# tobwei/APTAI

Hardware: AMD Instinct MI355X
Metric: utterances/sec (10 s @ 16 kHz) train-step (higher is better)
Workload: dtype bf16

## Files before the change

### aptai_amd/csrc/gemm.hip

```cpp
#include <stdlib.h>

#include <mutex>
#include <set>
#include <type_traits>

#include "common.h"
#include "gemm_common.h"

using namespace aptai_gemm;

namespace {

#ifdef APTAI_STAMPS
__device__ unsigned long long g_stamps[4096 * 8];
#define APTAI_STAMP(slot)                                                                          \
    do {                                                                                           \
        if (threadIdx.x == 0 && blockIdx.x < 4096 && blockIdx.y == 0 && blockIdx.z == 0)           \
            g_stamps[blockIdx.x * 8 + (slot)] = wall_clock64();                                    \
    } while (0)
extern "C" int aptai_debug_read_stamps(void* host_out) {
    return hipMemcpyFromSymbol(host_out, HIP_SYMBOL(g_stamps), sizeof(g_stamps)) == hipSuccess ? 0 : 1;
}
#else
#define APTAI_STAMP(slot) do {} while (0)
#endif

void epi_trace(const GemmArgs& g, int tile) {
    static const bool on = getenv("APTAI_EPI_TRACE") != nullptr;
    if (!on) return;
    static std::mutex mu;
    static std::set<int> seen;
    const int w = g.flags | (g.out_pre ? EPX_PRE : 0) | (g.colscale_n > 0 ? EPX_CS : 0);
    std::lock_guard<std::mutex> lk(mu);
    if (!seen.insert(w).second) return;
    bool listed = false;
#define APTAI_EPI_CASE(W) listed = listed || (w == (W));
    APTAI_EPI_WORDS(APTAI_EPI_CASE)
#undef APTAI_EPI_CASE
    fprintf(stderr, "[aptai epi] flag word 0x%x (tile %d, %d x %d x %d): %s\n", w, tile, g.M, g.N, g.K, listed ? "compiled" : "RUN-TIME form");
}

template <bool A_KM, bool B_KM, bool OUT_F32, int BM_T = 128, bool ROWSUM = false>
__device__ __forceinline__ void gemm_tile_body(GemmArgs g, const int bid, const int batch, const int split, float* rowsum = nullptr) {
    extern __shared__ __attribute__((aligned(16))) char smem[];
    APTAI_STAMP(0);
    const int tid = threadIdx.x;
    const int lane = tid & 63;
    const int wave = __builtin_amdgcn_readfirstlane(tid >> 6);
    const int wm = wave >> 1, wn = wave & 1;

    int tile_m, tile_n;
    raster2d(bid, g.tiles_m, g.tiles_n, g.raster_gm, tile_m, tile_n);
    constexpr int NI = BM_T / 32;
    constexpr int WM = BM_T / 2;
    constexpr int NA_IT = BM_T / 32;
    constexpr int A_BYTES_T = BM_T * BK * 2;
    constexpr int STAGE_T = A_BYTES_T + BN * BK * 2;
    constexpr int NPASS = BM_T / 16;
    static_assert(BM_T == 128 || (BM_T == 64 && !A_KM), "64-row tiles are built for K-contiguous A only");
    constexpr bool RING5 = A_KM && B_KM;
    const int m0 = tile_m * BM_T, n0 = tile_n * BN;

    if (batch >= 0) batch_offset<OUT_F32>(g, batch / g.nb_inner, batch % g.nb_inner);
    const auto [kt_begin, nk] = splitk_range(g, split);

    f32x4 acc[NI][4];
#pragma unroll
    for (int i = 0; i < NI; ++i)
#pragma unroll
        for (int j = 0; j < 4; ++j) acc[i][j] = (f32x4){0.f, 0.f, 0.f, 0.f};

    static_assert(!ROWSUM || (RING5 && OUT_F32), "row sums ride on the ring loop of the K-major fp32 weight-gradient tile");
    const bool rs_wave = ROWSUM && rowsum != nullptr && tile_n == 0 && wn == 0;
    const bf16x8 ones8 = __builtin_bit_cast(bf16x8, (short8v){0x3f80, 0x3f80, 0x3f80, 0x3f80, 0x3f80, 0x3f80, 0x3f80, 0x3f80});
    f32x4 racc[ROWSUM ? NI : 1];
#pragma unroll
    for (int i = 0; i < (ROWSUM ? NI : 1); ++i) racc[i] = (f32x4){0.f, 0.f, 0.f, 0.f};

    const int wave_base_tid = wave * 64;
    const bool wave_active = (m0 + wm * WM < g.M) && (n0 + wn * 64 < g.N);
    const bf16_t* pa[NA_IT];
    const bf16_t* pb[4];
    const long stepA = A_KM ? (long)BK * g.lda : (long)BK, stepB = B_KM ? (long)BK * g.ldb : (long)BK;
#pragma unroll
    for (int it = 0; it < NA_IT; ++it) pa[it] = stage_src<A_KM>(g.A, g.lda, m0, g.M, it, tid) + kt_begin * stepA;
#pragma unroll
    for (int it = 0; it < 4; ++it) pb[it] = stage_src<B_KM>(g.B, g.ldb, n0, g.N, it, tid) + kt_begin * stepB;
    auto stage = [&](char* buf) {
        char* dst = buf + wave_base_tid * 16;
#pragma unroll
        for (int it = 0; it < NA_IT; ++it) {
            __builtin_amdgcn_global_load_lds(GLB_PTR(pa[it]), LDS_PTR(dst + it * (NTHREADS * 16)), 16, 0, 0);
            pa[it] += stepA;
        }
#pragma unroll
        for (int it = 0; it < 4; ++it) {
            __builtin_amdgcn_global_load_lds(GLB_PTR(pb[it]), LDS_PTR(dst + A_BYTES_T + it * (NTHREADS * 16)), 16, 0, 0);
            pb[it] += stepB;
        }
    };
    if constexpr (RING5) {
        constexpr int HALF_T = RING_HALF_BYTES;
        const bf16_t* ha[2];
        const bf16_t* hb[2];
        const long hstepA = 32 * (long)g.lda, hstepB = 32 * (long)g.ldb;
#pragma unroll
        for (int it = 0; it < 2; ++it) {
// ... 650 lines not shown
        int cfirst = c - 1;
        while (cfirst > 0 && (int)((unsigned)cfirst * (unsigned)total / (unsigned)G) > tile * KT) --cfirst;
        if (tid == 0) {
            bool ok = true;
            for (int cp = cfirst; cp < c && ok; ++cp) {
                unsigned spins = 0;
                while (__hip_atomic_load(sk.flags + cp, __ATOMIC_RELAXED, __HIP_MEMORY_SCOPE_AGENT) == 0u) {
                    if (++spins > SK_SPIN_LIMIT) { atomicExch(sk.status, 1u); ok = false; break; }
                    __builtin_amdgcn_s_sleep(2);
                }
            }
            __builtin_amdgcn_fence(__ATOMIC_ACQUIRE, "agent");
            asm volatile("s_waitcnt vmcnt(0)" ::: "memory");
        }
        __syncthreads();
        {
            constexpr int QI = 8;
            const int nq = 4 * (c - cfirst);
            auto issue_quarter = [&](int q) {
                const float* slab = sk.slabs + (long)(cfirst + (q >> 2)) * SK_SLAB_FLOATS;
                char* dst = smem + (q & 1) * (QI * T2_THREADS * 16);
#pragma unroll
                for (int e = 0; e < QI; ++e) {
                    const int idx = (q & 3) * QI + e;
                    __builtin_amdgcn_global_load_lds(GLB_PTR(slab + ((long)idx * T2_THREADS + tid) * 4),
                                                     LDS_PTR(dst + (e * T2_THREADS + wave_base_tid) * 16), 16, 0, 0);
                }
            };
            issue_quarter(0);
            if (nq > 1) issue_quarter(1);
            for (int q = 0; q < nq; ++q) {
                if (q + 1 < nq) asm volatile("s_waitcnt vmcnt(8)" ::: "memory");
                else asm volatile("s_waitcnt vmcnt(0)" ::: "memory");
                const char* src = smem + (q & 1) * (QI * T2_THREADS * 16);
                f32x4 part[QI];
#pragma unroll
                for (int e = 0; e < QI; ++e) part[e] = *(const f32x4*)(src + (e * T2_THREADS + tid) * 16);
                asm volatile("s_waitcnt lgkmcnt(0)" ::: "memory");
                if (q + 2 < nq) issue_quarter(q + 2);
#pragma unroll
                for (int a = 0; a < 2; ++a)
#pragma unroll
                    for (int b = 0; b < 2; ++b)
#pragma unroll
                        for (int i = 0; i < 4; ++i)
#pragma unroll
                            for (int j = 0; j < 2; ++j) {
                                const int idx = ((a * 2 + b) * 4 + i) * 2 + j;
                                if ((idx >> 3) == (q & 3)) acc[a][b][i][j] += part[idx & 7];
                            }
            }
            __syncthreads();
        }
        if (tid == 0)
            for (int cp = cfirst; cp < c; ++cp) __hip_atomic_store(sk.flags + cp, 0u, __ATOMIC_RELAXED, __HIP_MEMORY_SCOPE_AGENT);
        gemm256_epilogue<OUT_F32>(g, smem, m0, n0, 0, acc, tid, lane, wr, wc);
    }
}

constexpr int SK_MAX_GRID = 256;
constexpr int64_t SK_HEADER_BYTES = 4096;
static inline int64_t sk_workspace_bytes() { return SK_HEADER_BYTES + (int64_t)SK_MAX_GRID * SK_SLAB_FLOATS * 4; }

template <bool A_KM, bool B_KM, bool OUT_F32>
int launch_gemm256_sk(const GemmArgs& g, void* ws, hipStream_t stream) {
    SkArgs sk;
    sk.status = (unsigned*)ws;
    sk.flags = (unsigned*)((char*)ws + 256);
    sk.slabs = (float*)((char*)ws + SK_HEADER_BYTES);
    sk.kt_per_tile = g.K / BK;
    const long total = (long)g.tiles_m * g.tiles_n * sk.kt_per_tile;
    if (total >= (1L << 23)) APTAI_FAIL(APTAI_ERR_INVALID, "aptai_gemm_bf16: stream-K iteration count %ld out of range", total);
    sk.total_iters = (int)total;
    const int grid = total < SK_MAX_GRID ? (int)total : SK_MAX_GRID;
    return launch_kernel<gemm256_sk_kernel<A_KM, B_KM, OUT_F32>>({T2_THREADS, T2_SMEM, "gemm256_sk_kernel"}, dim3(grid), stream, g, sk);
}

constexpr int T3_THREADS = 512;
constexpr int T3_BM = 128, T3_BN = 192;
constexpr int T3_A_BYTES = T3_BM * BK * 2;
constexpr int T3_B_BYTES = T3_BN * BK * 2;
constexpr int T3_STAGE = T3_A_BYTES + T3_B_BYTES;
constexpr int T3_SMEM = 3 * T3_STAGE;
constexpr int T3_EPI_PITCH = T3_BN * 4 + 16;
static_assert(T3_BM * T3_EPI_PITCH <= T3_SMEM, "epilogue tile must fit the staging LDS");

__device__ __forceinline__ int pn_swz(int krow) { return (((krow >> 1) & 1) | (((krow >> 3) & 1) << 1)) << 1; }

template <bool KM>
__device__ __forceinline__ const bf16_t* stage3_src(const bf16_t* __restrict__ base, long ld, int row0, int rows_total, int it,
                                                    int tid) {
    if (!KM) {
        const int slot = it * T3_THREADS + tid, row = slot >> 3, pc = slot & 7;
        int grow = row0 + row;
        grow = grow < rows_total ? grow : rows_total - 1;
        return base + (long)grow * ld + ((pc ^ (row & 7)) << 3);
    } else {
        const int krow = tid >> 3, pc = tid & 7;
        int col = row0 + it * 64 + ((pc ^ pn_swz(krow)) << 3);
        col = col <= rows_total - 8 ? col : rows_total - 8;
        return base + (long)krow * ld + col;
    }
}

template <bool KM>
__device__ __forceinline__ bf16x8 read_frag3(const char* lds_tile, int row_base, int ks, int lane) {
    if (!KM) {
        return read_frag(lds_tile, row_base, ks, lane);
    } else {
        const char* panel = lds_tile + (row_base >> 6) * 8192;
        const int rb = row_base & 63;
        const int gq = lane >> 4, i = lane & 15, qq = i >> 2, p = i & 3;
        const int ch = (rb >> 3) + (p >> 1);
        const int sub = (p & 1) << 3;
        const int k_lo = ks * 32 + gq * 8 + qq;
        const int k_hi = k_lo + 4;
        const char* a0 = panel + k_lo * 128 + ((ch ^ pn_swz(k_lo)) << 4) + sub;
        const char* a1 = panel + k_hi * 128 + ((ch ^ pn_swz(k_hi)) << 4) + sub;
        short4v lo = __builtin_amdgcn_ds_read_tr16_b64_v4i16((__attribute__((address_space(3))) short4v*)a0);
        short4v hi = __builtin_amdgcn_ds_read_tr16_b64_v4i16((__attribute__((address_space(3))) short4v*)a1);
        short8v r = {lo[0], lo[1], lo[2], lo[3], hi[0], hi[1], hi[2], hi[3]};
        return __builtin_bit_cast(bf16x8, r);
    }
}

template <bool A_KM, bool B_KM, bool OUT_F32>
__global__ __launch_bounds__(T3_THREADS, 1) void gemm192_kernel(GemmArgs g) {
    extern __shared__ __attribute__((aligned(16))) char smem[];
    APTAI_STAMP(0);
    const int tid = threadIdx.x;
    const int lane = tid & 63;
    const int wave = __builtin_amdgcn_readfirstlane(tid >> 6);
    const int wm = wave >> 2, wn = wave & 3;
    const int wave_base_tid = wave * 64;

    const int nwg = g.tiles_m * g.tiles_n;
    const int bid = xcd_remap(blockIdx.x, nwg);
    int tile_m, tile_n;
    raster2d(bid, g.tiles_m, g.tiles_n, g.raster_gm, tile_m, tile_n);
    const int m0 = tile_m * T3_BM, n0 = tile_n * T3_BN;
    if (gridDim.y > 1) batch_offset<OUT_F32>(g, blockIdx.y / g.nb_inner, blockIdx.y % g.nb_inner);
    const int split = blockIdx.z;
    const auto [kt_begin, nk] = splitk_range(g, split);

    const bf16_t* pa[2];
    const bf16_t* pb[3];
    const long stepA = A_KM ? (long)BK * g.lda : (long)BK;
    const long stepB = B_KM ? (long)BK * g.ldb : (long)BK;
#pragma unroll
    for (int it = 0; it < 2; ++it) pa[it] = stage3_src<A_KM>(g.A, g.lda, m0, g.M, it, tid) + (long)kt_begin * stepA;
#pragma unroll
    for (int it = 0; it < 3; ++it) pb[it] = stage3_src<B_KM>(g.B, g.ldb, n0, g.N, it, tid) + (long)kt_begin * stepB;
    auto stage = [&](int slot) {
        char* buf = smem + slot * T3_STAGE + wave_base_tid * 16;
#pragma unroll
        for (int it = 0; it < 2; ++it) {
            __builtin_amdgcn_global_load_lds(GLB_PTR(pa[it]), LDS_PTR(buf + it * (T3_THREADS * 16)), 16, 0, 0);
            pa[it] += stepA;
        }
#pragma unroll
        for (int it = 0; it < 3; ++it) {
            __builtin_amdgcn_global_load_lds(GLB_PTR(pb[it]), LDS_PTR(buf + T3_A_BYTES + it * (T3_THREADS * 16)), 16, 0, 0);
            pb[it] += stepB;
        }
    };

    f32x4 acc[4][3];
#pragma unroll
    for (int i = 0; i < 4; ++i)
#pragma unroll
        for (int j = 0; j < 3; ++j) acc[i][j] = (f32x4){0.f, 0.f, 0.f, 0.f};

    if constexpr (!A_KM && B_KM) {
        u32x4 aa[2][4];
        short4v bl[2][3], bh[2][3];
        auto read_half = [&](int slot, int ks) {
            const char* sa = smem + slot * T3_STAGE;
            const char* sb = sa + T3_A_BYTES;
#pragma unroll
            for (int i = 0; i < 4; ++i) {
                const int row = wm * 64 + i * 16 + (lane & 15), q = ks * 4 + (lane >> 4);
                const uint32_t addr = lds_u32(sa) + (uint32_t)(row * 128 + ((q ^ (row & 7)) << 4));
                asm volatile("ds_read_b128 %0, %1" : "=v"(aa[ks][i]) : "v"(addr));
            }
#pragma unroll
            for (int j = 0; j < 3; ++j) {
                const int row_base = wn * 48 + j * 16;
                const char* panel = sb + (row_base >> 6) * 8192;
                const int rb = row_base & 63;
                const int gq = lane >> 4, li = lane & 15, qq = li >> 2, pp = li & 3;
                const int ch = (rb >> 3) + (pp >> 1);
                const int sub = (pp & 1) << 3;
                const int k_lo = ks * 32 + gq * 8 + qq, k_hi = k_lo + 4;
                const uint32_t a0 = lds_u32(panel) + (uint32_t)(k_lo * 128 + ((ch ^ pn_swz(k_lo)) << 4) + sub);
                const uint32_t a1 = lds_u32(panel) + (uint32_t)(k_hi * 128 + ((ch ^ pn_swz(k_hi)) << 4) + sub);
                asm volatile("ds_read_b64_tr_b16 %0, %1" : "=v"(bl[ks][j]) : "v"(a0));
                asm volatile("ds_read_b64_tr_b16 %0, %1" : "=v"(bh[ks][j]) : "v"(a1));
            }
        };
        auto mfma_half = [&](int ks) {
#pragma unroll
            for (int i = 0; i < 4; ++i)
#pragma unroll
                for (int j = 0; j < 3; ++j)
                    acc[i][j] = __builtin_amdgcn_mfma_f32_16x16x32_bf16(combine_tr(bl[ks][j], bh[ks][j]), __builtin_bit_cast(bf16x8, aa[ks][i]),
                                                                        acc[i][j], 0, 0, 0);
        };
#define APTAI_TIE_HALF(K) "+v"(aa[K][0]), "+v"(aa[K][1]), "+v"(aa[K][2]), "+v"(aa[K][3]), "+v"(bl[K][0]), "+v"(bl[K][1]), "+v"(bl[K][2]), \
                          "+v"(bh[K][0]), "+v"(bh[K][1]), "+v"(bh[K][2])
        if (nk > 0) {
            stage(0);
            if (nk > 1) stage(1);
            if (nk > 2) stage(2);
            if (nk > 2) asm volatile("s_waitcnt vmcnt(10)" ::: "memory");
            else if (nk > 1) asm volatile("s_waitcnt vmcnt(5)" ::: "memory");
            else asm volatile("s_waitcnt vmcnt(0)" ::: "memory");
            __builtin_amdgcn_s_barrier();
            asm volatile("" ::: "memory");
            read_half(0, 0);
            read_half(0, 1);
        }
        int cur = 0;
        for (int kt = 0; kt < nk; ++kt) {
            const int nxt = cur == 2 ? 0 : cur + 1;
            asm volatile("s_waitcnt lgkmcnt(10)" : APTAI_TIE_HALF(0));
            mfma_half(0);
            if (kt + 1 < nk) {
                if (kt + 2 < nk) asm volatile("s_waitcnt vmcnt(5) lgkmcnt(0)" ::: "memory");
                else asm volatile("s_waitcnt vmcnt(0) lgkmcnt(0)" ::: "memory");
                __builtin_amdgcn_s_barrier();
                asm volatile("" ::: "memory");
                if (kt + 3 < nk) stage(cur);
                asm volatile("" : APTAI_TIE_HALF(1));
                read_half(nxt, 0);
            } else {
                asm volatile("s_waitcnt lgkmcnt(0)" : APTAI_TIE_HALF(1));
            }
            mfma_half(1);
            if (kt + 1 < nk) read_half(nxt, 1);
            cur = nxt;
        }
#undef APTAI_TIE_HALF
    } else {
    bf16x8 af[2][4], bfr[2][3];
    auto read_half = [&](int slot, int ks) {
        const char* sa = smem + slot * T3_STAGE;
        const char* sb = sa + T3_A_BYTES;
#pragma unroll
        for (int i = 0; i < 4; ++i) af[ks][i] = read_frag3<A_KM>(sa, wm * 64 + i * 16, ks, lane);
#pragma unroll
        for (int j = 0; j < 3; ++j) bfr[ks][j] = read_frag3<B_KM>(sb, wn * 48 + j * 16, ks, lane);
    };
    auto mfma_half = [&](int ks) {
#pragma unroll
        for (int i = 0; i < 4; ++i)
#pragma unroll
            for (int j = 0; j < 3; ++j)
                acc[i][j] = __builtin_amdgcn_mfma_f32_16x16x32_bf16(bfr[ks][j], af[ks][i], acc[i][j], 0, 0, 0);
    };

    if (nk > 0) {
        stage(0);
        if (nk > 1) stage(1);
        if (nk > 2) stage(2);
        if (nk > 2) asm volatile("s_waitcnt vmcnt(10)" ::: "memory");
        else if (nk > 1) asm volatile("s_waitcnt vmcnt(5)" ::: "memory");
        else asm volatile("s_waitcnt vmcnt(0)" ::: "memory");
        __builtin_amdgcn_s_barrier();
        asm volatile("" ::: "memory");
        read_half(0, 0);
        read_half(0, 1);
    }
    int cur = 0;
#ifdef APTAI_STAMPS
    unsigned long long seg[5] = {0, 0, 0, 0, 0}, tp = __builtin_amdgcn_s_memtime();
#define SEG(i) do { const unsigned long long tn = __builtin_amdgcn_s_memtime(); seg[i] += tn - tp; tp = tn; } while (0)
#else
#define SEG(i) do {} while (0)
#endif
    for (int kt = 0; kt < nk; ++kt) {
        const int nxt = cur == 2 ? 0 : cur + 1;
        mfma_half(0);
        SEG(0);
        if (kt + 1 < nk) {
            if (kt + 2 < nk) asm volatile("s_waitcnt vmcnt(5) lgkmcnt(0)" ::: "memory");
            else asm volatile("s_waitcnt vmcnt(0) lgkmcnt(0)" ::: "memory");
            __builtin_amdgcn_s_barrier();
            asm volatile("" ::: "memory");
            SEG(1);
            if (kt + 3 < nk) stage(cur);
            read_half(nxt, 0);
            SEG(2);
        }
        mfma_half(1);
        SEG(3);
        if (kt + 1 < nk) read_half(nxt, 1);
        SEG(4);
        cur = nxt;
    }
#ifdef APTAI_STAMPS
    if (threadIdx.x == 0 && blockIdx.x < 4096 && blockIdx.y == 0 && blockIdx.z == 0) {
        g_stamps[blockIdx.x * 8 + 1] = seg[0];
        g_stamps[blockIdx.x * 8 + 5] = seg[1];
        g_stamps[blockIdx.x * 8 + 6] = seg[2];
        g_stamps[blockIdx.x * 8 + 7] = seg[3] | (seg[4] << 32);
    }
#endif
#undef SEG
    }
    asm volatile("s_waitcnt vmcnt(0) lgkmcnt(0)" ::: "memory");
    __syncthreads();

    APTAI_STAMP(2);
    int tid_e, lane_e, m0_e, n0_e;
    epi_idx(tid, lane, m0, n0, tid_e, lane_e, m0_e, n0_e);
    const int fx = epi_flag_word(g);
    auto body = [&](auto w) {
        constexpr int FM = decltype(w)::value;
        const int flags = FM >= 0 ? FM : fx;
        u32x4 resv[6], auxv[6];
    #pragma unroll
        for (int pass = 0; pass < 6; ++pass) {
            resv[pass] = (u32x4){0u, 0u, 0u, 0u};
            auxv[pass] = (u32x4){0u, 0u, 0u, 0u};
        }
        if (!OUT_F32 && (flags & (APTAI_EPI_RESIDUAL | APTAI_EPI_DGELU | APTAI_EPI_MUL_AUX))) {
    #pragma unroll
            for (int pass = 0; pass < 6; ++pass) {
                const int c = pass * T3_THREADS + tid_e, ml = c / 24, cl = (c - ml * 24) * 8;
                int m = m0_e + ml, n = n0_e + cl;
                m = m < g.M ? m : g.M - 1;
                n = n <= g.N - 8 ? n : g.N - 8;
                if (flags & APTAI_EPI_RESIDUAL) resv[pass] = *(const u32x4*)(g.residual + (long)m * g.ldr + n);
                if (flags & (APTAI_EPI_DGELU | APTAI_EPI_MUL_AUX)) auxv[pass] = *(const u32x4*)(g.aux + (long)m * g.ldaux + n);
            }
        }
    #pragma unroll
        for (int i = 0; i < 4; ++i) {
            const int ml = wm * 64 + i * 16 + (lane_e & 15);
    #pragma unroll
            for (int j = 0; j < 3; ++j) {
                const int nl = wn * 48 + j * 16 + (lane_e >> 4) * 4;
                *(f32x4*)(smem + ml * T3_EPI_PITCH + nl * 4) = acc[i][j];
            }
        }
        __syncthreads();
        const float alpha = (flags & APTAI_EPI_ALPHA) ? g.alpha : 1.0f;
        uint32_t sd0 = g.seed0, sd1 = g.seed1;
        if (flags & APTAI_EPI_DROPOUT) apply_salt(g.salt, sd0, sd1);
    #pragma unroll
        for (int pass = 0; pass < 6; ++pass) {
            const int c = pass * T3_THREADS + tid_e, ml = c / 24, cl = (c - ml * 24) * 8;
            const int m = m0_e + ml, n = n0_e + cl;
            if (m >= g.M || n >= g.N) continue;
            const f32x4 v0 = *(const f32x4*)(smem + ml * T3_EPI_PITCH + cl * 4);
            const f32x4 v1 = *(const f32x4*)(smem + ml * T3_EPI_PITCH + cl * 4 + 16);
            float v[8] = {v0[0], v0[1], v0[2], v0[3], v1[0], v1[1], v1[2], v1[3]};
            if (flags & APTAI_EPI_BIAS) {
                const f32x4 b0 = *(const f32x4*)(g.bias + n), b1 = *(const f32x4*)(g.bias + n + 4);
    #pragma unroll
                for (int r = 0; r < 4; ++r) { v[r] = fmaf(v[r], alpha, b0[r]); v[4 + r] = fmaf(v[4 + r], alpha, b1[r]); }
            } else if (flags & APTAI_EPI_ALPHA) {
    #pragma unroll
                for (int r = 0; r < 8; ++r) v[r] *= alpha;
            }
            if (OUT_F32) {
                store_f32_tail(g, flags, v, m, n, split);
                continue;
            }
            epilogue_chunk<FM>(v, g, flags, (long)m, n, auxv[pass], resv[pass], sd0, sd1);
            __builtin_amdgcn_sched_barrier(0);
        }
    };
    if (OUT_F32) body(EpiWord<-1>{});
    else epi_dispatch(fx, body);
    APTAI_STAMP(3);
#ifdef APTAI_STAMPS
    asm volatile("s_waitcnt vmcnt(0)" ::: "memory");
    APTAI_STAMP(4);
#endif
}

}


struct GemmKnobs {
    int tile;
    double f256;
    int m64;
    int raster;
    bool splitn;
    bool epi_runtime;
};
static const GemmKnobs& gemm_knobs() {
    static const auto env = [](const char* name, const char* unset) { const char* e = getenv(name); return e ? e : unset; };
    static const GemmKnobs k = {atoi(env("APTAI_GEMM_TILE", "0")), atof(env("APTAI_GEMM_F256", "1.25")), atoi(env("APTAI_GEMM_M64", "1")),
                                atoi(env("APTAI_GEMM_RASTER", "-1")), atoi(env("APTAI_GEMM_SPLITN", "0")) != 0 && !getenv("APTAI_GEMM_TILE"),
                                atoi(env("APTAI_EPI_RUNTIME", "0")) != 0};
    return k;
}
static int raster_group(const GemmKnobs& k, int entry_default) { return k.raster >= 0 ? k.raster : entry_default; }

struct GemmPlan : aptai_gemm_plan_info { const char* refusal; };
static constexpr int tile_rows(int t) { return t == 64 ? 64 : (t == 256 || t == 257) ? T2_BM : t == 448 ? 256 : t == 192 ? T3_BM : BM; }
static constexpr int tile_cols(int t) { return t == 192 ? T3_BN : (t == 256 || t == 257) ? T2_BN : t == 448 ? 192 : BN; }
static void launch_shape(const aptai_gemm_desc& d, int& nbatch, int& nsplit, int& ktiles_per_split) {
    nbatch = (d.batch_outer > 1 || d.batch_inner > 1) ? (d.batch_outer > 0 ? d.batch_outer : 1) * (d.batch_inner > 0 ? d.batch_inner : 1) : 1;
    const int total_kt = (int)(d.K / BK);
    nsplit = d.split_k > 0 ? (d.split_k < total_kt ? d.split_k : total_kt) : 1;
    ktiles_per_split = (int)ceil_div(total_kt, nsplit);
    nsplit = (int)ceil_div(total_kt, ktiles_per_split);
}

static int validate_desc(const aptai_gemm_desc* d) {
    APTAI_REQUIRE(d != nullptr, "aptai_gemm_bf16: null descriptor");
    APTAI_REQUIRE(d->M > 0 && d->N > 0 && d->K > 0, "aptai_gemm_bf16: empty problem M=%ld N=%ld K=%ld", (long)d->M,
                  (long)d->N, (long)d->K);
    APTAI_REQUIRE(d->K % BK == 0, "aptai_gemm_bf16: K=%ld must be a multiple of %d", (long)d->K, BK);
    APTAI_REQUIRE(d->N % 8 == 0, "aptai_gemm_bf16: N=%ld must be a multiple of 8", (long)d->N);
    APTAI_REQUIRE(d->A && d->B && d->C, "aptai_gemm_bf16: null operand");
    APTAI_REQUIRE(d->lda % 8 == 0 && d->ldb % 8 == 0 && d->ldc % 8 == 0, "aptai_gemm_bf16: leading dims must keep 16-B alignment");
    if (d->residual) APTAI_REQUIRE(d->ldr % 8 == 0 && (uintptr_t)d->residual % 16 == 0, "aptai_gemm_bf16: residual must be 16-B aligned");
    if (d->aux) APTAI_REQUIRE(d->ldaux % 8 == 0 && (uintptr_t)d->aux % 16 == 0, "aptai_gemm_bf16: aux must be 16-B aligned");
    if (d->bias) APTAI_REQUIRE((uintptr_t)d->bias % 16 == 0, "aptai_gemm_bf16: bias must be 16-B aligned");
    APTAI_REQUIRE(((uintptr_t)d->A % 16 == 0) && ((uintptr_t)d->B % 16 == 0) && ((uintptr_t)d->C % 16 == 0),
                  "aptai_gemm_bf16: operands must be 16-byte aligned");
    if (d->a_kmajor) APTAI_REQUIRE(d->M % 8 == 0 && d->M >= 8, "aptai_gemm_bf16: K-major A needs M %% 8 == 0");
    if (d->b_kmajor) APTAI_REQUIRE(d->N >= 8, "aptai_gemm_bf16: K-major B needs N >= 8");
    if (d->flags & APTAI_EPI_BIAS) APTAI_REQUIRE(d->bias != nullptr, "aptai_gemm_bf16: EPI_BIAS without bias");
    if (d->flags & APTAI_EPI_RESIDUAL) APTAI_REQUIRE(d->residual != nullptr, "aptai_gemm_bf16: EPI_RESIDUAL without residual");
    if (d->flags & APTAI_EPI_RESIDUAL_F32)
        APTAI_REQUIRE(d->residual != nullptr && d->out_f32 && !(d->flags & APTAI_EPI_RESIDUAL) && d->split_k <= 1 && !d->accumulate &&
                      (d->tile == 128 || d->tile == 64 || d->tile == 192 || d->tile == 256 || d->tile == 257),
                      "aptai_gemm_bf16: EPI_RESIDUAL_F32 needs fp32 output, a residual, no split-K / accumulate and an explicit tile");
    if (d->flags & (APTAI_EPI_DGELU | APTAI_EPI_MUL_AUX)) APTAI_REQUIRE(d->aux != nullptr, "aptai_gemm_bf16: EPI_DGELU / EPI_MUL_AUX without aux");
    if (d->flags & APTAI_EPI_PRE_DGELU) APTAI_REQUIRE(d->out_pre != nullptr && (d->flags & APTAI_EPI_GELU), "aptai_gemm_bf16: EPI_PRE_DGELU needs EPI_GELU and out_pre");

    if (d->flags & APTAI_EPI_BIAS_ROW)
        APTAI_REQUIRE(d->out_f32 && d->bias != nullptr && !(d->flags & APTAI_EPI_BIAS) && (d->tile == 128 || d->tile == 192 || d->tile == 256) &&
                      d->split_k <= 1 && !d->accumulate, "aptai_gemm_bf16: EPI_BIAS_ROW needs out_f32, a bias of length M, no EPI_BIAS, tile 128 / 192 / 256");
    if (d->flags & APTAI_EPI_SPLIT_OUT)
        APTAI_REQUIRE(d->out_f32 && (d->tile == 128 || d->tile == 192 || d->tile == 256) && !d->a_kmajor && d->split_k <= 1 && !d->accumulate && (d->split_out_pieces == 3 || d->split_out_pieces == 6) &&
                      d->ldc >= d->split_out_pieces * d->N && d->N % 8 == 0,
                      "aptai_gemm_bf16: EPI_SPLIT_OUT needs out_f32, tile 128 / 192 / 256, 3 or 6 pieces and ldc >= pieces * N (bf16 elements)");
    APTAI_REQUIRE(d->colscale_n >= 0 && d->colscale_n % 8 == 0 && d->colscale_n <= d->N && (d->colscale_n == 0 || !d->out_f32),
                  "aptai_gemm_bf16: colscale_n must be a multiple of 8 within N, bf16 output only");
    int nbatch, nsplit, ktiles_per_split;
    launch_shape(*d, nbatch, nsplit, ktiles_per_split);
    if (nbatch > 1) {
        for (int l = 0; l < 2; ++l)
            APTAI_REQUIRE(d->batch_stride_a[l] % 8 == 0 && d->batch_stride_b[l] % 8 == 0 && d->batch_stride_c[l] % 8 == 0 &&
                              d->batch_stride_bias[l] % 4 == 0 && d->batch_stride_res[l] % 8 == 0 && d->batch_stride_aux[l] % 8 == 0,
                          "aptai_gemm_bf16: batch strides must keep vector alignment");
        APTAI_REQUIRE(nbatch <= 65535, "aptai_gemm_bf16: too many batches");
    }
    const bool f32 = d->out_f32 != 0;
    if (nbatch > 1) APTAI_REQUIRE(!(f32 && (d->split_k > 1 || d->accumulate)), "aptai_gemm_bf16: batched GEMM cannot split-K/accumulate");
    if (!f32) APTAI_REQUIRE(nsplit == 1, "aptai_gemm_bf16: split-K needs fp32 output");
    if (f32 && (nsplit > 1 || d->accumulate)) {
        APTAI_REQUIRE(d->workspace != nullptr, "aptai_gemm_bf16: split-K / accumulate needs a workspace");
        APTAI_REQUIRE(d->ldc == d->N, "aptai_gemm_bf16: split-K output must be dense (ldc == N)");
        APTAI_REQUIRE((size_t)d->workspace_bytes >= (size_t)nsplit * d->M * d->N * 4, "aptai_gemm_bf16: workspace too small");
// ... 224 lines not shown
```

Baseline: 1766.

## Prefetch residual during GEMM192 mainloop tail and pipeline epilogue LDS reads

For the A-row-major/B-K-major gemm192 path, the main K loop is split into a steady part and a tail part. The residual tile loads are issued as raw global loads before the last three K tiles, and the counted vmcnt waits are adjusted so the residual is fetched while the final MFMAs run instead of after them. The epilogue also software-pipelines its LDS reads of the next chunk. The intent is to hide residual-load latency in residual-fused epilogues. The cost is fragile hand-counted waitcnt values and extra register pressure from six held residual vectors. Stamp instrumentation is added only under APTAI_STAMPS.

Result: no change. 1779, median of 6 (+0.8%).

```diff
diff --git a/aptai_amd/csrc/gemm.hip b/aptai_amd/csrc/gemm.hip
--- a/aptai_amd/csrc/gemm.hip
+++ b/aptai_amd/csrc/gemm.hip
@@ -21,8 +21,20 @@
 extern "C" int aptai_debug_read_stamps(void* host_out) {
     return hipMemcpyFromSymbol(host_out, HIP_SYMBOL(g_stamps), sizeof(g_stamps)) == hipSuccess ? 0 : 1;
 }
+#define APTAI_STAMP_REG(var)                                                                       \
+    do {                                                                                           \
+        var = wall_clock64();                                                                      \
+        asm volatile("s_waitcnt lgkmcnt(0)" ::: "memory");                                         \
+    } while (0)
+#define APTAI_STAMP_FLUSH(slot, var)                                                               \
+    do {                                                                                           \
+        if (threadIdx.x == 0 && blockIdx.x < 4096 && blockIdx.y == 0 && blockIdx.z == 0)           \
+            g_stamps[blockIdx.x * 8 + (slot)] = var;                                               \
+    } while (0)
 #else
 #define APTAI_STAMP(slot) do {} while (0)
+#define APTAI_STAMP_REG(var) do {} while (0)
+#define APTAI_STAMP_FLUSH(slot, var) do {} while (0)
 #endif
 
 void epi_trace(const GemmArgs& g, int tile) {
@@ -839,6 +851,8 @@
 constexpr int T3_B_BYTES = T3_BN * BK * 2;
 constexpr int T3_STAGE = T3_A_BYTES + T3_B_BYTES;
 constexpr int T3_SMEM = 3 * T3_STAGE;
+constexpr int T3_NPF = T3_BM * T3_BN / 8 / T3_THREADS;
+static_assert(T3_NPF == 6, "the counted waits of gemm192_kernel spell 5 + 6, 10 + 6, 0 + 6");
 constexpr int T3_EPI_PITCH = T3_BN * 4 + 16;
 static_assert(T3_BM * T3_EPI_PITCH <= T3_SMEM, "epilogue tile must fit the staging LDS");
 
@@ -885,6 +899,9 @@
 __global__ __launch_bounds__(T3_THREADS, 1) void gemm192_kernel(GemmArgs g) {
     extern __shared__ __attribute__((aligned(16))) char smem[];
     APTAI_STAMP(0);
+#ifdef APTAI_STAMPS
+    unsigned long long t_dma0 = 0, t_mfma0 = 0, t_store0 = 0;
+#endif
     const int tid = threadIdx.x;
     const int lane = tid & 63;
     const int wave = __builtin_amdgcn_readfirstlane(tid >> 6);
@@ -898,7 +915,8 @@
     const int m0 = tile_m * T3_BM, n0 = tile_n * T3_BN;
     if (gridDim.y > 1) batch_offset<OUT_F32>(g, blockIdx.y / g.nb_inner, blockIdx.y % g.nb_inner);
     const int split = blockIdx.z;
-    const auto [kt_begin, nk] = splitk_range(g, split);
+    const KRange kr = splitk_range(g, split);
+    const int kt_begin = kr.kt_begin, nk = kr.nk;
 
     const bf16_t* pa[2];
     const bf16_t* pb[3];
@@ -927,6 +945,55 @@
     for (int i = 0; i < 4; ++i)
 #pragma unroll
         for (int j = 0; j < 3; ++j) acc[i][j] = (f32x4){0.f, 0.f, 0.f, 0.f};
+
+    constexpr bool SPLIT_LOOP = !A_KM && B_KM;
+    const bool pre_res = SPLIT_LOOP && !OUT_F32 && (g.flags & APTAI_EPI_RESIDUAL) != 0;
+    u32x4 resq[T3_NPF];
+#pragma unroll
+    for (int pass = 0; pass < T3_NPF; ++pass) resq[pass] = (u32x4){0u, 0u, 0u, 0u};
+    auto prefetch_res = [&]() {
+        asm volatile("" ::: "memory");
+#pragma unroll
+        for (int pass = 0; pass < T3_NPF; ++pass) {
+            const int c = pass * T3_THREADS + tid, ml = c / 24, cl = (c - ml * 24) * 8;
+            int m = m0 + ml, n = n0 + cl;
+            m = m < g.M ? m : g.M - 1;
+            n = n <= g.N - 8 ? n : g.N - 8;
+            const bf16_t* src = g.residual + (long)m * g.ldr + n;
+            asm volatile("global_load_dwordx4 %0, %1, off" : "+v"(resq[pass]) : "v"(src) : "memory");
+        }
+    };
+    auto prologue = [&]() {
+        if (nk > 0) stage(0);
+        if (nk > 1) stage(1);
+        if (nk > 2) stage(2);
+        const bool pf = pre_res && nk <= 3;
+        if (pf) prefetch_res();
+        APTAI_STAMP_REG(t_dma0);
+        if (nk > 2) {
+            if (pf) asm volatile("s_waitcnt vmcnt(16)" ::: "memory");
+            else asm volatile("s_waitcnt vmcnt(10)" ::: "memory");
+        } else if (nk > 1) {
+            if (pf) asm volatile("s_waitcnt vmcnt(11)" ::: "memory");
+            else asm volatile("s_waitcnt vmcnt(5)" ::: "memory");
+        } else {
+            if (pf) asm volatile("s_waitcnt vmcnt(6)" ::: "memory");
+            else asm volatile("s_waitcnt vmcnt(0)" ::: "memory");
+        }
+        __builtin_amdgcn_s_barrier();
+        asm volatile("" ::: "memory");
+    };
+    auto wait_tail = [&](int kt) {
+        if (kt + 2 < nk) {
+            if (pre_res) asm volatile("s_waitcnt vmcnt(11) lgkmcnt(0)" ::: "memory");
+            else asm volatile("s_waitcnt vmcnt(5) lgkmcnt(0)" ::: "memory");
+        } else {
+            if (pre_res) asm volatile("s_waitcnt vmcnt(6) lgkmcnt(0)" ::: "memory");
+            else asm volatile("s_waitcnt vmcnt(0) lgkmcnt(0)" ::: "memory");
+        }
+    };
+    using Steady = std::true_type;
+    using Tail = std::false_type;
 
     if constexpr (!A_KM && B_KM) {
         u32x4 aa[2][4];
@@ -965,36 +1032,40 @@
         };
 #define APTAI_TIE_HALF(K) "+v"(aa[K][0]), "+v"(aa[K][1]), "+v"(aa[K][2]), "+v"(aa[K][3]), "+v"(bl[K][0]), "+v"(bl[K][1]), "+v"(bl[K][2]), \
                           "+v"(bh[K][0]), "+v"(bh[K][1]), "+v"(bh[K][2])
+        prologue();
         if (nk > 0) {
-            stage(0);
-            if (nk > 1) stage(1);
-            if (nk > 2) stage(2);
-            if (nk > 2) asm volatile("s_waitcnt vmcnt(10)" ::: "memory");
-            else if (nk > 1) asm volatile("s_waitcnt vmcnt(5)" ::: "memory");
-            else asm volatile("s_waitcnt vmcnt(0)" ::: "memory");
-            __builtin_amdgcn_s_barrier();
-            asm volatile("" ::: "memory");
             read_half(0, 0);
             read_half(0, 1);
         }
-        int cur = 0;
-        for (int kt = 0; kt < nk; ++kt) {
-            const int nxt = cur == 2 ? 0 : cur + 1;
+        APTAI_STAMP_REG(t_mfma0);
+        auto ktile = [&](auto part, const int kt, const int cur, const int nxt) {
+            constexpr bool STEADY = decltype(part)::value;
             asm volatile("s_waitcnt lgkmcnt(10)" : APTAI_TIE_HALF(0));
             mfma_half(0);
-            if (kt + 1 < nk) {
-                if (kt + 2 < nk) asm volatile("s_waitcnt vmcnt(5) lgkmcnt(0)" ::: "memory");
-                else asm volatile("s_waitcnt vmcnt(0) lgkmcnt(0)" ::: "memory");
+            if (STEADY || kt + 1 < nk) {
+                if constexpr (STEADY) asm volatile("s_waitcnt vmcnt(5) lgkmcnt(0)" ::: "memory");
+                else wait_tail(kt);
                 __builtin_amdgcn_s_barrier();
                 asm volatile("" ::: "memory");
-                if (kt + 3 < nk) stage(cur);
+                if constexpr (STEADY) stage(cur);
                 asm volatile("" : APTAI_TIE_HALF(1));
                 read_half(nxt, 0);
             } else {
                 asm volatile("s_waitcnt lgkmcnt(0)" : APTAI_TIE_HALF(1));
             }
             mfma_half(1);
-            if (kt + 1 < nk) read_half(nxt, 1);
+            if (STEADY || kt + 1 < nk) read_half(nxt, 1);
+        };
+        int cur = 0, kt = 0;
+        for (; kt + 3 < nk; ++kt) {
+            const int nxt = cur == 2 ? 0 : cur + 1;
+            ktile(Steady{}, kt, cur, nxt);
+            cur = nxt;
+        }
+        if (pre_res && nk > 3) prefetch_res();
+        for (; kt < nk; ++kt) {
+            const int nxt = cur == 2 ? 0 : cur + 1;
+            ktile(Tail{}, kt, cur, nxt);
             cur = nxt;
         }
 #undef APTAI_TIE_HALF
@@ -1020,6 +1091,7 @@
         stage(0);
         if (nk > 1) stage(1);
         if (nk > 2) stage(2);
+        APTAI_STAMP_REG(t_dma0);
         if (nk > 2) asm volatile("s_waitcnt vmcnt(10)" ::: "memory");
         else if (nk > 1) asm volatile("s_waitcnt vmcnt(5)" ::: "memory");
         else asm volatile("s_waitcnt vmcnt(0)" ::: "memory");
@@ -1028,8 +1100,9 @@
         read_half(0, 0);
         read_half(0, 1);
     }
+    APTAI_STAMP_REG(t_mfma0);
     int cur = 0;
-#ifdef APTAI_STAMPS
+#if APTAI_STAMPS + 0 >= 2
     unsigned long long seg[5] = {0, 0, 0, 0, 0}, tp = __builtin_amdgcn_s_memtime();
 #define SEG(i) do { const unsigned long long tn = __builtin_amdgcn_s_memtime(); seg[i] += tn - tp; tp = tn; } while (0)
 #else
@@ -1055,7 +1128,7 @@
         SEG(4);
         cur = nxt;
     }
-#ifdef APTAI_STAMPS
+#if APTAI_STAMPS + 0 >= 2
     if (threadIdx.x == 0 && blockIdx.x < 4096 && blockIdx.y == 0 && blockIdx.z == 0) {
         g_stamps[blockIdx.x * 8 + 1] = seg[0];
         g_stamps[blockIdx.x * 8 + 5] = seg[1];
@@ -1065,7 +1138,8 @@
 #endif
 #undef SEG
     }
-    asm volatile("s_waitcnt vmcnt(0) lgkmcnt(0)" ::: "memory");
+    asm volatile("s_waitcnt vmcnt(0) lgkmcnt(0)"
+                 : "+v"(resq[0]), "+v"(resq[1]), "+v"(resq[2]), "+v"(resq[3]), "+v"(resq[4]), "+v"(resq[5])::"memory");
     __syncthreads();
 
     APTAI_STAMP(2);
@@ -1081,14 +1155,14 @@
             resv[pass] = (u32x4){0u, 0u, 0u, 0u};
             auxv[pass] = (u32x4){0u, 0u, 0u, 0u};
         }
-        if (!OUT_F32 && (flags & (APTAI_EPI_RESIDUAL | APTAI_EPI_DGELU | APTAI_EPI_MUL_AUX))) {
+        if (!OUT_F32 && (flags & ((SPLIT_LOOP ? 0 : APTAI_EPI_RESIDUAL) | APTAI_EPI_DGELU | APTAI_EPI_MUL_AUX))) {
     #pragma unroll
             for (int pass = 0; pass < 6; ++pass) {
                 const int c = pass * T3_THREADS + tid_e, ml = c / 24, cl = (c - ml * 24) * 8;
                 int m = m0_e + ml, n = n0_e + cl;
                 m = m < g.M ? m : g.M - 1;
                 n = n <= g.N - 8 ? n : g.N - 8;
-                if (flags & APTAI_EPI_RESIDUAL) resv[pass] = *(const u32x4*)(g.residual + (long)m * g.ldr + n);
+                if (!SPLIT_LOOP && (flags & APTAI_EPI_RESIDUAL)) resv[pass] = *(const u32x4*)(g.residual + (long)m * g.ldr + n);
                 if (flags & (APTAI_EPI_DGELU | APTAI_EPI_MUL_AUX)) auxv[pass] = *(const u32x4*)(g.aux + (long)m * g.ldaux + n);
             }
         }
@@ -1105,13 +1179,30 @@
         const float alpha = (flags & APTAI_EPI_ALPHA) ? g.alpha : 1.0f;
         uint32_t sd0 = g.seed0, sd1 = g.seed1;
         if (flags & APTAI_EPI_DROPOUT) apply_salt(g.salt, sd0, sd1);
+        [[maybe_unused]] f32x4 nv0, nv1;
+        if constexpr (SPLIT_LOOP) {
+            const int ml = tid_e / 24, cl = (tid_e - ml * 24) * 8;
+            nv0 = *(const f32x4*)(smem + ml * T3_EPI_PITCH + cl * 4);
+            nv1 = *(const f32x4*)(smem + ml * T3_EPI_PITCH + cl * 4 + 16);
+        }
     #pragma unroll
         for (int pass = 0; pass < 6; ++pass) {
             const int c = pass * T3_THREADS + tid_e, ml = c / 24, cl = (c - ml * 24) * 8;
             const int m = m0_e + ml, n = n0_e + cl;
+            f32x4 v0, v1;
+            if constexpr (SPLIT_LOOP) {
+                v0 = nv0, v1 = nv1;
+                if (pass + 1 < 6) {
+                    const int c1 = c + T3_THREADS, ml1 = c1 / 24, cl1 = (c1 - ml1 * 24) * 8;
+                    nv0 = *(const f32x4*)(smem + ml1 * T3_EPI_PITCH + cl1 * 4);
+                    nv1 = *(const f32x4*)(smem + ml1 * T3_EPI_PITCH + cl1 * 4 + 16);
+                }
+            }
             if (m >= g.M || n >= g.N) continue;
-            const f32x4 v0 = *(const f32x4*)(smem + ml * T3_EPI_PITCH + cl * 4);
-            const f32x4 v1 = *(const f32x4*)(smem + ml * T3_EPI_PITCH + cl * 4 + 16);
+            if constexpr (!SPLIT_LOOP) {
+                v0 = *(const f32x4*)(smem + ml * T3_EPI_PITCH + cl * 4);
+                v1 = *(const f32x4*)(smem + ml * T3_EPI_PITCH + cl * 4 + 16);
+            }
             float v[8] = {v0[0], v0[1], v0[2], v0[3], v1[0], v1[1], v1[2], v1[3]};
             if (flags & APTAI_EPI_BIAS) {
                 const f32x4 b0 = *(const f32x4*)(g.bias + n), b1 = *(const f32x4*)(g.bias + n + 4);
@@ -1125,7 +1216,8 @@
                 store_f32_tail(g, flags, v, m, n, split);
                 continue;
             }
-            epilogue_chunk<FM>(v, g, flags, (long)m, n, auxv[pass], resv[pass], sd0, sd1);
+            epilogue_chunk<FM>(v, g, flags, (long)m, n, auxv[pass], SPLIT_LOOP ? resq[pass] : resv[pass], sd0, sd1);
+            if (pass == 0) APTAI_STAMP_REG(t_store0);
             __builtin_amdgcn_sched_barrier(0);
         }
     };
@@ -1135,6 +1227,11 @@
 #ifdef APTAI_STAMPS
     asm volatile("s_waitcnt vmcnt(0)" ::: "memory");
     APTAI_STAMP(4);
+#if APTAI_STAMPS + 0 == 1
+    APTAI_STAMP_FLUSH(1, t_mfma0);
+    APTAI_STAMP_FLUSH(5, t_store0);
+    APTAI_STAMP_FLUSH(6, t_dma0);
+#endif
 #endif
 }
 
```

## Split gemm192 row-major A path into two staggered wave groups with private A staging

Applied to the files above, without the earlier changes.

For the bf16-output, row-major A and K-major B case, the main loop now runs through a new routine. The eight waves form two groups of four. Each group stages its own 64-row half of A, all waves share the B tile, and the groups are offset by one barrier so one group's MFMAs can overlap the other's LDS reads. MFMA bursts run at raised priority via setprio, and a full tile is read from LDS before the compute. The prefetch depth becomes two tiles ahead instead of three, and optional timing instrumentation is added behind a compile flag. This adds barrier complexity and a shallower pipeline, in exchange for better overlap between LDS and MFMA work.

New measurement: 1752 before, 1757 after, median of 6. Within noise of the previous version (+0.3%).

```diff
diff --git a/aptai_amd/csrc/gemm.hip b/aptai_amd/csrc/gemm.hip
--- a/aptai_amd/csrc/gemm.hip
+++ b/aptai_amd/csrc/gemm.hip
@@ -881,6 +881,173 @@
     }
 }
 
+#ifdef APTAI_T3_STAMPS
+__device__ unsigned long long g_t3_seg[1024 * 2 * 16];
+#define T3_SEG_INIT()                                                                                   \
+    unsigned long long seg_[16], tp_, rt0_;                                                             \
+    for (int q_ = 0; q_ < 16; ++q_) seg_[q_] = 0;                                                       \
+    __builtin_amdgcn_sched_barrier(0);                                                                  \
+    asm volatile("s_memrealtime %0\n\ts_waitcnt lgkmcnt(0)" : "=s"(rt0_)::"memory");                     \
+    asm volatile("s_memtime %0\n\ts_waitcnt lgkmcnt(0)" : "=s"(tp_)::"memory");                          \
+    const unsigned long long t0_ = tp_;                                                                 \
+    __builtin_amdgcn_sched_barrier(0)
+#if APTAI_T3_STAMPS >= 2
+#define T3_SEG(i)                                                                                       \
+    do {                                                                                                \
+        unsigned long long tn_;                                                                         \
+        __builtin_amdgcn_sched_barrier(0);                                                              \
+        asm volatile("s_memtime %0\n\ts_waitcnt lgkmcnt(0)" : "=s"(tn_)::"memory");                      \
+        __builtin_amdgcn_sched_barrier(0);                                                              \
+        seg_[i] += tn_ - tp_;                                                                           \
+        tp_ = tn_;                                                                                      \
+    } while (0)
+#else
+#define T3_SEG(i) do {} while (0)
+#endif
+#define T3_SEG_DONE()                                                                                   \
+    do {                                                                                                \
+        unsigned long long rt1_, t1_;                                                                   \
+        __builtin_amdgcn_sched_barrier(0);                                                              \
+        asm volatile("s_memtime %0\n\ts_waitcnt lgkmcnt(0)" : "=s"(t1_)::"memory");                      \
+        asm volatile("s_memrealtime %0\n\ts_waitcnt lgkmcnt(0)" : "=s"(rt1_)::"memory");                 \
+        __builtin_amdgcn_sched_barrier(0);                                                              \
+        seg_[14] = t1_ - t0_;                                          \
+        seg_[15] = rt1_ - rt0_;                                        \
+        if ((threadIdx.x & 255) == 0 && blockIdx.x < 1024 && blockIdx.y == 0 && blockIdx.z == 0)        \
+            for (int q_ = 0; q_ < 16; ++q_) g_t3_seg[(blockIdx.x * 2 + (threadIdx.x >> 8)) * 16 + q_] = seg_[q_]; \
+    } while (0)
+extern "C" int aptai_debug_read_t3_stamps(void* host_out) {
+    return hipMemcpyFromSymbol(host_out, HIP_SYMBOL(g_t3_seg), sizeof(g_t3_seg)) == hipSuccess ? 0 : 1;
+}
+#else
+#define T3_SEG_INIT() do {} while (0)
+#define T3_SEG(i) do {} while (0)
+#define T3_SEG_DONE() do {} while (0)
+#endif
+
+constexpr int T3G_APART = 64 * BK * 2;
+constexpr int T3G_B0 = 2 * 3 * T3G_APART;
+static_assert(T3G_B0 + 3 * T3_B_BYTES <= T3_SMEM, "two-group staging must fit the allocation");
+
+__device__ __forceinline__ void t3_groups_mainloop(const GemmArgs& g, char* smem, const int m0, const int n0, const int kt_begin, const int nk,
+                                                   f32x4 (&acc)[4][3], const int tid, const int lane, const int wave) {
+    const int grp = wave >> 2, wn = wave & 3;
+    char* const sA = smem + grp * (3 * T3G_APART);
+    char* const sB = smem + T3G_B0;
+    const bf16_t* pa[2];
+    const bf16_t* pb[3];
+#pragma unroll
+    for (int it = 0; it < 2; ++it) {
+        const int cid = it * 256 + (tid & 255), row = cid >> 3, pc = cid & 7;
+        int grow = m0 + grp * 64 + row;
+        grow = grow < g.M ? grow : g.M - 1;
+        pa[it] = g.A + (long)grow * g.lda + (long)kt_begin * BK + ((pc ^ (row & 7)) << 3);
+    }
+    const long stepB = (long)BK * g.ldb;
+#pragma unroll
+    for (int it = 0; it < 3; ++it) pb[it] = stage3_src<true>(g.B, g.ldb, n0, g.N, it, tid) + (long)kt_begin * stepB;
+    auto stage = [&](int slot) {
+        char* dA = sA + slot * T3G_APART + wn * 1024;
+        char* dB = sB + slot * T3_B_BYTES + wave * 1024;
+#pragma unroll
+        for (int it = 0; it < 2; ++it) {
+            __builtin_amdgcn_global_load_lds(GLB_PTR(pa[it]), LDS_PTR(dA + it * 4096), 16, 0, 0);
+            pa[it] += BK;
+        }
+#pragma unroll
+        for (int it = 0; it < 3; ++it) {
+            __builtin_amdgcn_global_load_lds(GLB_PTR(pb[it]), LDS_PTR(dB + it * 8192), 16, 0, 0);
+            pb[it] += stepB;
+        }
+    };
+
+    u32x4 aa[2][4];
+    short4v bl[2][3], bh[2][3];
+    auto read_tile = [&](const char* tA, const char* tB) {
+#pragma unroll
+        for (int ks = 0; ks < 2; ++ks) {
+#pragma unroll
+            for (int j = 0; j < 3; ++j) {
+                const int row_base = wn * 48 + j * 16;
+                const char* panel = tB + (row_base >> 6) * 8192;
+                const int rb = row_base & 63;
+                const int gq = lane >> 4, li = lane & 15, qq = li >> 2, pp = li & 3;
+                const int ch = (rb >> 3) + (pp >> 1);
+                const int sub = (pp & 1) << 3;
+                const int k_lo = ks * 32 + gq * 8 + qq, k_hi = k_lo + 4;
+                const uint32_t a0 = lds_u32(panel) + (uint32_t)(k_lo * 128 + ((ch ^ pn_swz(k_lo)) << 4) + sub);
+                const uint32_t a1 = lds_u32(panel) + (uint32_t)(k_hi * 128 + ((ch ^ pn_swz(k_hi)) << 4) + sub);
+                asm volatile("ds_read_b64_tr_b16 %0, %1" : "=v"(bl[ks][j]) : "v"(a0));
+                asm volatile("ds_read_b64_tr_b16 %0, %1" : "=v"(bh[ks][j]) : "v"(a1));
+            }
+#pragma unroll
+            for (int i = 0; i < 4; ++i) {
+                const int row = i * 16 + (lane & 15), q = ks * 4 + (lane >> 4);
+                const uint32_t addr = lds_u32(tA) + (uint32_t)(row * 128 + ((q ^ (row & 7)) << 4));
+                asm volatile("ds_read_b128 %0, %1" : "=v"(aa[ks][i]) : "v"(addr));
+            }
+        }
+    };
+#define APTAI_TIE_HALF(K) "+v"(aa[K][0]), "+v"(aa[K][1]), "+v"(aa[K][2]), "+v"(aa[K][3]), "+v"(bl[K][0]), "+v"(bl[K][1]), "+v"(bl[K][2]), \
+                          "+v"(bh[K][0]), "+v"(bh[K][1]), "+v"(bh[K][2])
+
+    stage(0);
+    if (nk > 1) {
+        stage(1);
+        asm volatile("s_waitcnt vmcnt(5)" ::: "memory");
+    } else {
+        asm volatile("s_waitcnt vmcnt(0)" ::: "memory");
+    }
+    __builtin_amdgcn_s_barrier();
+    if (grp == 1) __builtin_amdgcn_s_barrier();
+    asm volatile("" ::: "memory");
+
+    int slot = 0;
+    T3_SEG_INIT();
+    for (int t = 0; t < nk; ++t) {
+        read_tile(sA + slot * T3G_APART, sB + slot * T3_B_BYTES);
+        __builtin_amdgcn_sched_barrier(0);
+        T3_SEG(0);
+        if (t + 2 < nk) {
+            stage(slot == 0 ? 2 : slot - 1);
+            T3_SEG(1);
+            asm volatile("s_waitcnt vmcnt(5)" ::: "memory");
+        } else {
+            T3_SEG(1);
+            if (t + 1 < nk) asm volatile("s_waitcnt vmcnt(0)" ::: "memory");
+        }
+        asm volatile("s_waitcnt lgkmcnt(0)" : APTAI_TIE_HALF(0)::"memory");
+        asm volatile("" : APTAI_TIE_HALF(1));
+        T3_SEG(2);
+        __builtin_amdgcn_s_barrier();
+        T3_SEG(3);
+        __builtin_amdgcn_sched_barrier(0);
+        __builtin_amdgcn_s_setprio(1);
+#pragma unroll
+        for (int ks = 0; ks < 2; ++ks)
+#pragma unroll
+            for (int i = 0; i < 4; ++i)
+#pragma unroll
+                for (int j = 0; j < 3; ++j)
+                    acc[i][j] = __builtin_amdgcn_mfma_f32_16x16x32_bf16(combine_tr(bl[ks][j], bh[ks][j]), __builtin_bit_cast(bf16x8, aa[ks][i]),
+                                                                        acc[i][j], 0, 0, 0);
+        __builtin_amdgcn_s_setprio(0);
+#pragma unroll
+        for (int i = 0; i < 4; ++i)
+#pragma unroll
+            for (int j = 0; j < 3; ++j) asm volatile("" : "+v"(acc[i][j]));
+        __builtin_amdgcn_sched_barrier(0);
+        T3_SEG(4);
+        __builtin_amdgcn_s_barrier();
+        asm volatile("" ::: "memory");
+        T3_SEG(5);
+        slot = slot == 2 ? 0 : slot + 1;
+    }
+    T3_SEG_DONE();
+#undef APTAI_TIE_HALF
+    if (grp == 0) __builtin_amdgcn_s_barrier();
+}
+
 template <bool A_KM, bool B_KM, bool OUT_F32>
 __global__ __launch_bounds__(T3_THREADS, 1) void gemm192_kernel(GemmArgs g) {
     extern __shared__ __attribute__((aligned(16))) char smem[];
@@ -928,7 +1095,9 @@
 #pragma unroll
         for (int j = 0; j < 3; ++j) acc[i][j] = (f32x4){0.f, 0.f, 0.f, 0.f};
 
-    if constexpr (!A_KM && B_KM) {
+    if constexpr (!A_KM && B_KM && !OUT_F32) {
+        t3_groups_mainloop(g, smem, m0, n0, kt_begin, nk, acc, tid, lane, wave);
+    } else if constexpr (!A_KM && B_KM) {
         u32x4 aa[2][4];
         short4v bl[2][3], bh[2][3];
         auto read_half = [&](int slot, int ks) {
@@ -978,6 +1147,7 @@
             read_half(0, 1);
         }
         int cur = 0;
+        T3_SEG_INIT();
         for (int kt = 0; kt < nk; ++kt) {
             const int nxt = cur == 2 ? 0 : cur + 1;
             asm volatile("s_waitcnt lgkmcnt(10)" : APTAI_TIE_HALF(0));
@@ -997,6 +1167,7 @@
             if (kt + 1 < nk) read_half(nxt, 1);
             cur = nxt;
         }
+        T3_SEG_DONE();
 #undef APTAI_TIE_HALF
     } else {
     bf16x8 af[2][4], bfr[2][3];
@@ -1029,6 +1200,7 @@
         read_half(0, 1);
     }
     int cur = 0;
+    T3_SEG_INIT();
 #ifdef APTAI_STAMPS
     unsigned long long seg[5] = {0, 0, 0, 0, 0}, tp = __builtin_amdgcn_s_memtime();
 #define SEG(i) do { const unsigned long long tn = __builtin_amdgcn_s_memtime(); seg[i] += tn - tp; tp = tn; } while (0)
@@ -1055,6 +1227,7 @@
         SEG(4);
         cur = nxt;
     }
+    T3_SEG_DONE();
 #ifdef APTAI_STAMPS
     if (threadIdx.x == 0 && blockIdx.x < 4096 && blockIdx.y == 0 && blockIdx.z == 0) {
         g_stamps[blockIdx.x * 8 + 1] = seg[0];
```
